# xultaeculcis/climate-super-resolution

Measured on NVIDIA B200. Metric: generator_inference_hr_mpixel_per_s, higher is better.
Workload: dtype bf16

## Files before the change

climate-super-resolution_b200/csrc/api.cu:

```cuda
#include <algorithm>
#include <atomic>
#include <cstdarg>
#include <cstdio>
#include <cstring>
#include <map>
#include <mutex>
#include <string>
#include <vector>

#include "../../include/climsr_b200.h"
#include "conv_tc.cuh"
#include "disc.cuh"
#include "elementwise.cuh"
#include "loss.cuh"
#include "metrics.cuh"
#include "rcan.cuh"
#include "rdb_tc.cuh"
#include "wgrad_tc.cuh"

namespace csr {

static thread_local char g_err[512] = "";
static std::atomic<long long> g_launches{0};
static int g_opt_pdl = 1;
// ... 9 lines not shown
static int g_opt_graphs = 1;
static int g_opt_graph_max_px = 1 << 21;
static int g_opt_wgrad_atomic = 1;
static int g_opt_eight_acc = 1;
static int g_opt_tall = 1;
static int g_opt_narrow_box = 1;
static int g_opt_trace_cta = 0;
static int g_opt_reserve_sms = 0;
static int g_opt_dense_min = 2;
static int g_opt_tap_pack = 1;
static int g_opt_hyb = 1;
static int g_opt_merge_phases = 1;
static int g_opt_fuse_tail = 3;
static int g_opt_dense = 1;
static int g_opt_early = 1;
static int g_dbg_wgrad[5] = {0, 0, 0, 0, 0};

static int fail(int code, const char* fmt, ...) {
  va_list ap;
  va_start(ap, fmt);
  vsnprintf(g_err, sizeof(g_err), fmt, ap);
  va_end(ap);
  return code;
}
#define CSR_CUDA(expr)                                                                          \
  do {                                                                                          \
    cudaError_t _e = (expr);                                                                    \
    if (_e != cudaSuccess) return fail(CSR_ERR_CUDA, "%s: %s", #expr, cudaGetErrorString(_e)); \
  } while (0)

// ... 160 lines not shown
        off = align_up(off + pp.npad * 4, 128);
        pl.parts.push_back(pp);
      }
    }
    out.push_back(pl);
  }
  *total = off;
  return out;
}

struct Tiling {
  int SW, TH, TW, win_rows, win_bytes, slot_bytes, n_slots, stage_bytes;
  double eff;
};
static int choose_tiling(int H, int W, int KH, int KW, int w_bytes, int n_kblocks, int stage_row_bytes, int n_stage, Tiling* out,
                         int row_bytes = 128, int tall = 1, int extra_slot_bytes = 0) {
  double best = -1;
  for (int SW = 16; SW <= 128; SW *= 2) {
    if (g_opt_force_sw && SW != g_opt_force_sw) continue;
    if (KW > 1 && SW > 32) continue;
    const int TW = SW - (KW - 1);
    if (TW < 1) continue;
    const int TH = kTileM / SW;
    const int win_rows = tall * TH + KH - 1;
    const int win_bytes = win_rows * SW * row_bytes;
    const int slot_bytes = (int)align_up(win_bytes, 1024) + (int)align_up(extra_slot_bytes, 1024);
    const int stage_bytes = stage_row_bytes ? (int)align_up((size_t)TH * TW * stage_row_bytes, 1024) : 0;
    const int fixed = 1024 + (int)align_up(w_bytes, 128) + 256 + 512 + n_stage * stage_bytes;
    const int slots = std::min(g_opt_max_slots, (kSmemLimit - fixed) / slot_bytes);
    if (slots < 1) continue;
    const double tiles = (double)ceil_div(H, TH * tall) * ceil_div(W, TW) * tall;
    double eff = (double)H * W / (tiles * kTileM);
    if (slots < std::min(2, n_kblocks + 1)) eff *= 0.7;
    eff -= 1e-4 * win_bytes / (double)(kTileM * 128);
    if (eff > best) {
      best = eff;
      *out = {SW, TH, TW, win_rows, win_bytes, slot_bytes, slots, stage_bytes, eff};
    }
  }
  if (best < 0) return fail(CSR_ERR_UNSUPPORTED, "no tile shape fits shared memory (weights %d bytes, %dx%d kernel)", w_bytes, KH, KW);
  return CSR_OK;
}

struct ConvLaunch {
  ConvParams p;
  CUtensorMap tmap;
  size_t w_off = 0, b_off = 0;
  size_t w2_off = 0, b2_off = 0;
};

struct DenseLaunch {
  DenseParams p;
  CUtensorMap tmap;
  size_t w_off[kDenseMaxLayers], b_off[kDenseMaxLayers];
// ... 70 lines not shown
    if (ok2 && te2.n_slots >= want) stages = 2;
    else if (ok1 && (!ok2 || te1.n_slots > te2.n_slots)) stages = 1;
    else if (ok2) stages = 2;
    const Tiling& te = stages == 1 ? te1 : te2;
    if (stages && te.n_slots >= std::min(2, p.n_kblocks + 1)) {
      tl = te;
      p.early = 1;
      p.n_groups = 1;
      p.n_stage = stages;
      if (4 * p.KW * p.npad <= 512 && !g_opt_two_acc) p.n_acc = 4;
    }
  }
  if (g_opt_hyb && p.early && ((p.KW == 3 && p.PW == 1) || (p.KW == 2 && p.PW <= 1)) && p.box_c == 64 && !p.stream_w) {
    p.hyb = 1;
    if (4 * (p.KW - 1) * p.npad <= 512 && !g_opt_two_acc) p.n_acc = 4;
  }
  p.SW = tl.SW; p.TH = tl.TH; p.TW = tl.TW;
  p.sw_shift = 0;
  while ((1 << p.sw_shift) < p.SW) ++p.sw_shift;
  p.tiles_x = ceil_div(W, p.TW);
  p.tiles_y = ceil_div(H, p.TH << p.tall_shift);
  p.num_tiles = p.tiles_x * p.tiles_y * N;
  p.tiles_per_img = p.tiles_x * p.tiles_y;
  if ((long long)p.tiles_x * p.tiles_y * N >= (1 << 24) || p.tiles_per_img >= (1 << 16))
    return fail(CSR_ERR_UNSUPPORTED, "too many tiles (%d x %d x %d) for one launch", p.tiles_x, p.tiles_y, N);
  p.magic_img = ((1ull << 40) / (unsigned)p.tiles_per_img) + 1;
  p.magic_row = ((1ull << 40) / (unsigned)p.tiles_x) + 1;
  p.win_rows = tl.win_rows; p.win_bytes = tl.win_bytes; p.slot_bytes = tl.slot_bytes; p.n_slots = tl.n_slots;
  p.win_slot_bytes = (int)align_up(tl.win_bytes, 1024);
  p.stage_bytes = tl.stage_bytes;
// ... 444 lines not shown
  int wmax = 0;
  for (int k = 0; k < 4; ++k) {
    const PackLayer& pl = packs[li + k];
    if (pl.parts.size() != 1 || pl.parts[0].npad != 16 || pl.parts[0].kh != 3 || pl.parts[0].kw != 3 || pl.cin_pad != nf + k * gc)
      return fail(CSR_ERR_UNSUPPORTED, "dense-block kernel: unexpected pack layout");
    p.L[k].ksteps = pl.cin_pad / 16;
    p.L[k].n_kblocks = ceil_div(pl.cin_pad, 64);
    p.L[k].w_bytes = pl.parts[0].w_bytes;
    p.L[k].out_coff = nf + k * gc;
    p.L[k].gate_coff = nf + (3 - k) * gc;
    dl->w_off[k] = pl.parts[0].w_off; dl->b_off[k] = pl.parts[0].b_off;
    wmax = std::max(wmax, pl.parts[0].w_bytes);
  }
  p.wbuf_bytes = (int)align_up(wmax, 1024);
  Tiling tl;
  int rc = choose_tiling(H, W, 3, 3, 2 * p.wbuf_bytes, 2, 32, 4, &tl, 128, 2);
  if (rc) return rc;
  if (tl.n_slots < 3) return fail(CSR_ERR_UNSUPPORTED, "dense-block kernel: window ring too shallow");
  p.SW = tl.SW; p.TH = tl.TH; p.TW = tl.TW;
  while ((1 << p.sw_shift) < p.SW) ++p.sw_shift;
  p.tiles_x = ceil_div(W, p.TW); p.tiles_y = ceil_div(H, 2 * p.TH);
  p.tiles_per_img = p.tiles_x * p.tiles_y;
  p.num_tiles = p.tiles_per_img * N;
  if ((long long)p.tiles_per_img * N >= (1 << 24) || p.tiles_per_img >= (1 << 16)) return fail(CSR_ERR_UNSUPPORTED, "dense-block kernel: too many windows");
  p.magic_img = ((1ull << 40) / (unsigned)p.tiles_per_img) + 1;
  p.magic_row = ((1ull << 40) / (unsigned)p.tiles_x) + 1;
  p.win_bytes = tl.win_bytes; p.slot_bytes = tl.slot_bytes; p.n_slots = std::min(tl.n_slots, 8);
  p.stage_bytes = (int)align_up((size_t)p.TH * p.TW * 32, 1024);
  if (dense_smem_bytes(p) > (size_t)kSmemLimit) return fail(CSR_ERR_UNSUPPORTED, "dense-block kernel needs %zu bytes of shared memory", dense_smem_bytes(p));
  return encode_act_map(&dl->tmap, buf, N, H, W, C, p.SW, 2 * p.TH + 2, 64);
}

static bool dense_enabled(const CsrNetDesc& d) { return g_opt_dense && d.gc == 16 && !g_opt_force_generic; }

static bool try_dense(const CsrPlan* P, const std::vector<PackLayer>& packs, int li, int j, void* buf, const void* gate, Op* op) {
  const CsrNetDesc& d = P->net;
  if (!dense_enabled(d)) return false;
  const size_t per_block = (size_t)kDenseMaxLayers * P->N * ceil_div(P->h, 8) * ceil_div(P->w, 14);
  op->kind = Op::kDense;
  return build_dense(packs, li, P->N, P->h, P->w, buf, P->ccat, d.nf, d.gc, P->flags + (size_t)j * per_block, &op->dense, gate, gate ? P->ccat : 0) ==
             CSR_OK &&
         (size_t)op->dense.p.num_tiles * kDenseMaxLayers <= per_block && op->dense.p.num_tiles >= g_opt_dense_min * P->sms;
}

static int plan_build(CsrPlan* P, const WsPtrs& ws, const std::vector<LayerSpec>& layers) {
  const CsrNetDesc& d = P->net;
  const int N = P->N, h = P->h, w = P->w;
  auto cat = [&](int j) -> void* { return ws.cat[P->train ? j : j % 3]; };
  size_t total = 0;
  const std::vector<PackLayer> packs = pack_layout(fwd_exec_table(d, layers), &total);
  const int C = P->ccat, nf = d.nf, gc = d.gc;
  std::vector<Op>& ops = P->fwd;
  {
    Op op; op.kind = Op::kNchw; op.dst = ws.xin; op.N = N; op.C = d.in_channels; op.H = h; op.W = w;
    ops.push_back(op);
  }
  int li = 0;
// ... 391 lines not shown
    case 2: g_opt_force_sw = value; return CSR_OK;
    case 3: g_opt_max_slots = value < 1 ? 1 : value; return CSR_OK;
    case 4: g_opt_no_tma_store = value ? 1 : 0; return CSR_OK;
    case 5: g_opt_two_acc = value ? 1 : 0; return CSR_OK;
    case 6: g_opt_force_generic = value ? 1 : 0; return CSR_OK;
    case 7: g_opt_one_mma = value ? 1 : 0; return CSR_OK;
    case 11: g_opt_graphs = value ? 1 : 0; return CSR_OK;
    case 12: g_opt_graph_max_px = value; return CSR_OK;
    case 15: g_opt_trace_cta = value; return CSR_OK;
    case 17: g_opt_narrow_box = value ? 1 : 0; return CSR_OK;
    case 18: g_opt_tall = value ? 1 : 0; return CSR_OK;
    case 19: g_opt_eight_acc = value ? 1 : 0; return CSR_OK;
    case 20: case 21: case 22: case 23: case 24: g_dbg_wgrad[key - 20] = value; return CSR_OK;
    case 25: g_opt_wgrad_atomic = value ? 1 : 0; return CSR_OK;
    case 27: g_opt_dense = value ? 1 : 0; return CSR_OK;
    case 36: g_opt_tap_pack = value ? 1 : 0; return CSR_OK;
    case 35:
      if (value != 0 && value != 1) return fail(CSR_ERR_BAD_ARG, "option 35: 0 or 1");
      g_opt_hyb = value; return CSR_OK;
    case 34: g_opt_merge_phases = value ? 1 : 0; return CSR_OK;
    case 33: g_opt_fuse_tail = value & 3; return CSR_OK;
    case 31: if (value < 0 || value > 64) return fail(CSR_ERR_BAD_ARG, "option 31: windows per SM in [0, 64]"); g_opt_dense_min = value; return CSR_OK;
    case 30: g_opt_reserve_sms = value < 0 ? 0 : value; return CSR_OK;
    case 26:
      if (value != 0 && value != 1) return fail(CSR_ERR_BAD_ARG, "option 26: 0 or 1");
      g_opt_early = value; return CSR_OK;
    default: return fail(CSR_ERR_BAD_ARG, "unknown option key %d", key);
  }
}

// ... 766 lines not shown
```

climate-super-resolution_b200/csrc/conv_tc.cu:

```cuda
#include <cstdio>

#include "conv_tc.cuh"
#include "ptx.cuh"

namespace csr {

namespace {

#ifdef CSR_ENABLE_TRACE
#define CSR_TRACE(role, tile_it, ev)                                                                                  \
  do {                                                                                                                \
    if (p.trace && blockIdx.x == p.trace_cta && (tile_it) < 64) p.trace[((role) * 64 + (tile_it)) * 8 + (ev)] = clock64();      \
  } while (0)
#else
#define CSR_TRACE(role, tile_it, ev) do { } while (0)
#endif

struct Tile {
  int n, y0, x0;
};

__device__ __forceinline__ int fast_div(int t, unsigned long long magic) {
  return static_cast<int>((static_cast<unsigned long long>(static_cast<unsigned>(t)) * magic) >> 40);
}
// ... 32 lines not shown
#pragma unroll
    for (int j = 0; j < 8; ++j) s[j] = __uint_as_float(raw[j]);
  } else {
    const int src = (lane + delta) & 31;
#pragma unroll
    for (int j = 0; j < 8; ++j) s[j] = __uint_as_float(__shfl_sync(0xffffffffu, raw[j], src));
  }
#pragma unroll
  for (int j = 0; j < 8; j += 2) {
    const float2 t = __fadd2_rn(make_float2(acc[j], acc[j + 1]), make_float2(s[j], s[j + 1]));
    acc[j] = t.x;
    acc[j + 1] = t.y;
  }
}

__device__ __forceinline__ void fma_residual8(float (&v)[8], const uint4& r, float scale) {
  const uint32_t w[4] = {r.x, r.y, r.z, r.w};
#pragma unroll
  for (int i = 0; i < 4; ++i) {
    const float2 t = __ffma2_rn(make_float2(v[2 * i], v[2 * i + 1]), make_float2(scale, scale), make_float2(bf16lo(w[i]), bf16hi(w[i])));
    v[2 * i] = t.x;
    v[2 * i + 1] = t.y;
  }
}

__device__ __forceinline__ void gate8(float (&v)[8], const uint4& g, float neg) {
  const uint32_t w[4] = {g.x, g.y, g.z, g.w};
#pragma unroll
  for (int i = 0; i < 4; ++i) {
    v[2 * i] *= (bf16lo(w[i]) > 0.f) ? 1.f : neg;
    v[2 * i + 1] *= (bf16hi(w[i]) > 0.f) ? 1.f : neg;
  }
}

__device__ __forceinline__ uint4 ldg16(const void* base, size_t pix, int C, int coff) {
  return __ldg(reinterpret_cast<const uint4*>(reinterpret_cast<const __nv_bfloat16*>(base) + pix * C + coff));
}

}

template <int KW_T, int PW_T, int ACT_T, int RES_T, int ST_T, int TALL_T = 0, int EARLY_T = 0, int FUSE_T = 0, int HYB_T = 0>
__global__ void __launch_bounds__(kConvThreads, 1)
conv_tc_kernel(const ConvParams p, const __grid_constant__ CUtensorMap tmap) {
  static_assert(!HYB_T || EARLY_T, "hybrid tap fold: early-release epilogue only");
  extern __shared__ uint8_t smem_raw[];
  const uint32_t smem_base = (smem_u32(smem_raw) + 1023u) & ~1023u;
  const uint32_t slots_addr = smem_base;
  const uint32_t stage_addr = slots_addr + static_cast<uint32_t>(p.n_slots) * p.slot_bytes;
  const uint32_t w_addr = stage_addr + static_cast<uint32_t>(p.n_stage) * p.stage_bytes;
  const int w_local = p.stream_w ? 0 : p.w_bytes;
  const uint32_t w2_addr = w_addr + ((w_local + 127) & ~127);
  const uint32_t b2_addr = w2_addr + (FUSE_T ? static_cast<uint32_t>(p.w2_bytes) : 0u);
  const uint32_t bias_addr = b2_addr + (FUSE_T ? 128u : 0u);
  const uint32_t bar_addr = bias_addr + 256;
  const int S = p.n_slots;
  const int NA = p.n_acc;
  const int NG = p.n_groups;
  const int wpg = kEpilogueWarps / NG;
  auto bar_w = bar_addr;
// ... 72 lines not shown
        if (kb == 0 && lane == 0) CSR_TRACE(0, pit, 0);
        mbar_wait_spin(bar_a_empty(slot), phase ^ 1);
        if (kb == 0 && lane == 0) CSR_TRACE(0, pit, 1);
        if (elect_one()) {
          if (p.stream_w) {
            const int ks_here = min(4, (p.cin >> 4) - kb * 4);
            const int wbytes = p.KH * ks_here * (KW * p.npad) * 32;
            mbar_arrive_expect_tx(bar_a_full(slot), p.win_bytes + wbytes);
            const uint8_t* wsrc = reinterpret_cast<const uint8_t*>(p.wpk) + static_cast<size_t>(blockIdx.y) * p.part_w_bytes +
                                  static_cast<size_t>(kb) * p.wkb_bytes;
            const uint32_t wdst = slots_addr + slot * p.slot_bytes + p.win_slot_bytes;
            for (int off = 0; off < wbytes; off += 32768) bulk_load(wdst + off, wsrc + off, min(32768, wbytes - off), bar_a_full(slot));
          } else {
            mbar_arrive_expect_tx(bar_a_full(slot), p.win_bytes);
          }
          tma_load_4d(slots_addr + slot * p.slot_bytes, &tmap, bar_a_full(slot), p.cin_off + kb * 64, tl.x0 - p.PW, tl.y0 - ph_eff, tl.n);
        }
        __syncwarp();
        if (++slot == S) { slot = 0; phase ^= 1; }
      }
    }
  } else if (warp <= kMmaWarps) {
    if (warp > p.n_mma) goto done;
    const int mw = warp - 1;
    const uint32_t idesc = make_idesc_bf16(kTileM, nmma);
    const uint32_t b_step16 = static_cast<uint32_t>(nmma * 32) >> 4;
    const uint32_t kb_w16 = static_cast<uint32_t>(p.KH * 4) * b_step16;
    const uint32_t row_bytes = static_cast<uint32_t>(p.box_c) * 2u;
    const uint32_t row16 = static_cast<uint32_t>(p.SW) * (row_bytes >> 4);
    const uint32_t a_layout = p.box_c == 64 ? 2u : p.box_c == 32 ? 4u : 6u;
    const uint32_t a_hi = ((8u * row_bytes) >> 4) | (1u << 14) | (a_layout << 29);
// ... 90 lines not shown
    }
  } else {
    const int ew = warp - 1 - kMmaWarps;
    const int g = ew / wpg;
    const int wj = ew - g * wpg;
    const int lane_grp = warp & 3;
    const int sub = wj >> 2;
    const int cstep = wpg >> 2;
    const int gthreads = wpg * 32;
    const bool tracer = (ew == 0 && lane == 0);
    const int m = lane_grp * 32 + lane;
    const int ty = m >> p.sw_shift;
    const int tx = m & (p.SW - 1);
    const int n_chunks = ST_T == 3 ? 1 : p.npad >> 3;
    const int PW = KW_T ? PW_T : p.PW;
    const bool col_ok = (tx >= PW) && (tx < PW + p.TW);
    const int srow = ty * p.TW + (tx - PW);
    const int act = ACT_T >= 0 ? ACT_T : p.act;
    const bool has_r1 = RES_T >= 0 ? (RES_T & 1) != 0 : p.r1 != nullptr;
    const bool has_r2 = RES_T >= 0 ? (RES_T & 2) != 0 : p.r2 != nullptr;
    const bool has_gate = RES_T >= 0 ? (RES_T & 4) != 0 : p.gate != nullptr;
    const bool tma_store = ST_T >= 0 ? ST_T == 1 : (p.store_mode == kStoreStaged);
    const bool need_pix = !tma_store || has_r1 || has_r2 || has_gate;
    const uint32_t swz = (p.stage_row_bytes == 128) ? static_cast<uint32_t>(srow & 7) : 0u;
    const uint32_t srow_addr = stage_addr + static_cast<uint32_t>(g) * p.stage_bytes + static_cast<uint32_t>(srow * p.stage_row_bytes);
    const uint32_t sbuf = stage_addr + static_cast<uint32_t>(g) * p.stage_bytes;
    const uint32_t t_lane = tmem_base + (static_cast<uint32_t>(lane_grp * 32) << 16);
    const int d0 = -PW, d1 = 1 - PW, d2 = 2 - PW;
    const int rp = p.stage_row_bytes >> 4;
    const int n_pieces = p.TH * p.TW * rp;
    uint32_t pc_s[4], pc_d[4], pc_yx[4];
    if (tma_store) {
      const int tid_g = wj * 32 + lane;
#pragma unroll
      for (int k = 0; k < 4; ++k) {
        const int i = tid_g + k * gthreads;
        const int sr = i / rp, c = i - sr * rp;
        const int dy = sr / p.TW, dx = sr - dy * p.TW;
        const uint32_t z = (p.stage_row_bytes == 128) ? static_cast<uint32_t>(sr & 7) : 0u;
        pc_s[k] = sbuf + static_cast<uint32_t>(sr * p.stage_row_bytes) + ((static_cast<uint32_t>(c) ^ z) << 4);
        pc_d[k] = static_cast<uint32_t>((dy * p.out_sy * p.out_W + dx * p.out_sx) * p.out_C + c * 8);
// ... 149 lines not shown
        }
      }
    } else
    for (int it = g; ; it += NG) {
      const int t = blockIdx.x + (it >> TALL_T) * static_cast<int>(gridDim.x);
      if (t >= p.num_tiles) break;
      if (tracer) CSR_TRACE(2, it, 3);
      Tile tl = decode_tile<TALL_T>(p, t);
      if constexpr (TALL_T) tl.y0 += (it & 1) * p.TH;
      bool valid = false;
      size_t pix = 0;
      int y = 0, x = 0;
      uint4 q1[4], q2[4];
      if (need_pix) {
        y = tl.y0 + ty;
        x = tl.x0 - PW + tx;
        valid = col_ok && (y < p.H) && (x < p.W);
        pix = (static_cast<size_t>(tl.n) * p.H + y) * p.W + x;
#pragma unroll
        for (int j = 0; j < 4; ++j) {
          const int ch0 = (2 * (sub + (j >> 1) * cstep) + (j & 1)) * 8;
          const bool on = valid && (ch0 < p.n_store);
          q1[j] = (on && has_r1) ? ldg16(p.r1, pix, p.r1_C, p.r1_coff + ch0) : make_uint4(0, 0, 0, 0);
          if (has_gate)
            q2[j] = (on && ch0 >= p.gate_from) ? ldg16(p.gate, pix, p.gate_C, p.gate_coff + ch0)
                                               : make_uint4(0x3f803f80u, 0x3f803f80u, 0x3f803f80u, 0x3f803f80u);
          else
            q2[j] = (on && has_r2) ? ldg16(p.r2, pix, p.r2_C, p.r2_coff + ch0) : make_uint4(0, 0, 0, 0);
        }
      }
      if (tma_store) named_bar_sync(1 + g, gthreads);
// ... 19 lines not shown
            tmem_ld_wait();
            gather_add8(v, r0, 0, lane);
          } else if constexpr (KW_T == 2) {
            uint32_t r0[8], r1[8];
            tmem_ld8(t_addr + ch0, r0);
            tmem_ld8(t_addr + p.npad + ch0, r1);
            tmem_ld_wait();
            gather_add8(v, r0, d0, lane);
            gather_add8(v, r1, d1, lane);
          } else if constexpr (KW_T == 3) {
            uint32_t r0[8], r1[8], r2[8];
            tmem_ld8(t_addr + ch0, r0);
            tmem_ld8(t_addr + p.npad + ch0, r1);
            tmem_ld8(t_addr + 2 * p.npad + ch0, r2);
            tmem_ld_wait();
            gather_add8(v, r0, d0, lane);
            gather_add8(v, r1, d1, lane);
            gather_add8(v, r2, d2, lane);
          } else {
            for (int dx = 0; dx < KW; ++dx) {
              uint32_t r[8];
              tmem_ld8(t_addr + dx * p.npad + ch0, r);
              tmem_ld_wait();
              gather_add8(v, r, dx - PW, lane);
            }
          }
          apply_act8(v, act, p.act_slope);
          if (need_pix) {
            if (has_r1) fma_residual8(v, q1[j], p.s1);
            if (has_gate) gate8(v, q2[j], p.gate_neg);
            else if (has_r2) fma_residual8(v, q2[j], p.s2);
          }
          if (tma_store) {
// ... 50 lines not shown
  __syncthreads();
  timeline_end(p.timeline, p.launch_id);
  if (warp == 1) {
    __syncwarp();
    tc_fence_after();
    tmem_dealloc(tmem_base, p.tmem_cols);
  }
}

size_t conv_smem_bytes(const ConvParams& p) {
  return 1024  + static_cast<size_t>(p.n_slots) * p.slot_bytes + static_cast<size_t>(p.n_stage) * p.stage_bytes +
         (((p.stream_w ? 0 : p.w_bytes) + 127) & ~127) + (p.fuse2 ? p.w2_bytes + 128 : 0) + 256  +
         8 * (18 + 2 * p.n_slots) + 32;
}

template <int KW_T, int PW_T, int ACT_T, int RES_T, int ST_T, int TALL_T = 0, int EARLY_T = 0, int FUSE_T = 0, int HYB_T = 0>
static int launch_t(const ConvParams& p, const CUtensorMap& tmap, int num_sms, cudaStream_t stream) {
  const size_t smem = conv_smem_bytes(p);
  if (smem > static_cast<size_t>(kSmemLimit)) return static_cast<int>(cudaErrorInvalidValue);
  static bool configured[64] = {};
  auto kern = conv_tc_kernel<KW_T, PW_T, ACT_T, RES_T, ST_T, TALL_T, EARLY_T, FUSE_T, HYB_T>;
  int dev = 0;
  if (cudaGetDevice(&dev) != cudaSuccess || dev < 0 || dev >= 64) return static_cast<int>(cudaErrorInvalidDevice);
  if (!configured[dev]) {
    cudaError_t e = cudaFuncSetAttribute(kern, cudaFuncAttributeMaxDynamicSharedMemorySize, kSmemLimit);
    if (e != cudaSuccess) return static_cast<int>(e);
    configured[dev] = true;
  }
  cudaLaunchConfig_t cfg{};
  const int parts = p.parts > 1 ? p.parts : 1;
  const int per_part = num_sms / parts > 0 ? num_sms / parts : 1;
  cfg.gridDim = dim3(p.num_tiles < per_part ? p.num_tiles : per_part, parts);
  cfg.blockDim = dim3(kConvThreads);
  cfg.dynamicSmemBytes = smem;
  cfg.stream = stream;
  cudaLaunchAttribute attr[1];
  attr[0].id = cudaLaunchAttributeProgrammaticStreamSerialization;
  attr[0].val.programmaticStreamSerializationAllowed = p.use_pdl ? 1 : 0;
  cfg.attrs = attr;
  cfg.numAttrs = 1;
  return static_cast<int>(cudaLaunchKernelEx(&cfg, kern, p, tmap));
}

int launch_conv_tc(const ConvParams& p, const CUtensorMap& tmap, int num_sms, cudaStream_t stream) {
  const int res = (p.r1 ? 1 : 0) | (p.r2 ? 2 : 0) | (p.gate ? 4 : 0);
  if ((res & 6) == 6) return static_cast<int>(cudaErrorInvalidValue);
  if (p.tall_shift) {
    if ((p.n_acc != 4 && p.n_acc != 8) || p.n_groups != 4) return static_cast<int>(cudaErrorInvalidValue);
    if (p.store_mode == kStoreStaged && !p.force_generic && p.KW == 3 && p.PW == 1 && p.act == 1 && res == 0)
      return launch_t<3, 1, 1, 0, 1, 1>(p, tmap, num_sms, stream);
    if (p.store_mode == kStoreStaged && !p.force_generic && p.KW == 1 && p.PW == 0 && p.act == 2 && res == 0)
      return launch_t<1, 0, 2, 0, 1, 1>(p, tmap, num_sms, stream);
    if (p.store_mode == kStoreStaged && !p.force_generic && p.KW == 3 && p.PW == 1 && p.act == 0 && res == 4)
      return launch_t<3, 1, 0, 4, 1, 1>(p, tmap, num_sms, stream);
    if (p.store_mode == kStoreStaged && !p.force_generic && p.KW == 3 && p.PW == 1 && p.act == 0 && res == 5)
      return launch_t<3, 1, 0, 5, 1, 1>(p, tmap, num_sms, stream);
    if (p.store_mode == kStoreStaged && !p.force_generic && p.KW == 1 && p.PW == 0 && p.act == 0 && res == 4)
      return launch_t<1, 0, 0, 4, 1, 1>(p, tmap, num_sms, stream);
    if (p.store_mode == kStoreF32Planar && !p.force_generic && p.KW == 3 && p.PW == 1 && p.act == 0 && res == 0)
      return launch_t<3, 1, 0, 0, 3, 1>(p, tmap, num_sms, stream);
    if (p.store_mode == kStoreF32Planar && !p.force_generic && p.KW == 5 && p.PW == 2 && p.act == 0 && res == 0)
// ... 67 lines not shown
```

climate-super-resolution_b200/csrc/conv_tc.cuh:

```cuda
#pragma once
#include <cuda.h>
#include <cuda_runtime.h>
#include <stdint.h>

namespace csr {

constexpr int kEpilogueWarps = 16;
constexpr int kEpilogueThreads = kEpilogueWarps * 32;
constexpr int kMmaWarps = 2;
constexpr int kConvThreads = 32 * (1 + kMmaWarps) + kEpilogueThreads;
constexpr int kTileM = 128;
constexpr int kSmemLimit = 232448;
constexpr int kMaxNpad = 64;

enum StoreMode {
  kStoreStaged = 0,
  kStoreDirect = 1,
  kStoreF32Planar = 2,
  kStoreF32Nhwc = 3
};

struct ConvParams {
  int N, H, W;
  int KH, KW, PH, PW;
// ... 13 lines not shown
  int n_mma;
  int n_acc;
  int n_groups;
  int n_stage;
  int hyb;
  int early;
  int tmem_cols;
  int force_generic;
  int trace_cta;
  int box_c;
  int tall_shift;
  int stream_w;
  int wkb_bytes;
  int win_slot_bytes;
  int use_pdl;
  int parts, part_w_bytes, part_b_floats, part_c;
  int part_ph, part_oy;
  int fuse2, w2_bytes, n2;
  const void* w2;
  const float* b2;
  void* out2; int out2_C, out2_coff;
  long long out2_plane;
  const float* bias;
  const void* wpk;
  int act;
  float act_slope;
  float s1, s2;
  const void* r1; int r1_C, r1_coff;
  const void* r2; int r2_C, r2_coff;
  const void* gate; int gate_C, gate_coff; int gate_from; float gate_neg;
// ... 17 lines not shown
```

climate-super-resolution_b200/csrc/rdb_tc.cu:

```cuda
#include <cstdio>

#include "conv_tc.cuh"
#include "ptx.cuh"
#include "rdb_tc.cuh"

namespace csr {

namespace {

constexpr int kNpad = 16;
constexpr int kNmma = 3 * kNpad;
constexpr int kAcc = 8;
constexpr int kGroups = 4;

struct Win {
  int n, y0, x0, ty, tx;
};

__device__ __forceinline__ int fast_div(int t, unsigned long long magic) {
  return static_cast<int>((static_cast<unsigned long long>(static_cast<unsigned>(t)) * magic) >> 40);
}
__device__ __forceinline__ Win decode_win(const DenseParams& p, int t) {
  Win r;
  r.n = fast_div(t, p.magic_img);
// ... 26 lines not shown
#pragma unroll
    for (int j = 0; j < 8; ++j) s[j] = __uint_as_float(raw[j]);
  } else {
    const int src = (lane + delta) & 31;
#pragma unroll
    for (int j = 0; j < 8; ++j) s[j] = __uint_as_float(__shfl_sync(0xffffffffu, raw[j], src));
  }
#pragma unroll
  for (int j = 0; j < 8; j += 2) {
    const float2 t = __fadd2_rn(make_float2(acc[j], acc[j + 1]), make_float2(s[j], s[j + 1]));
    acc[j] = t.x;
    acc[j + 1] = t.y;
  }
}

}

__global__ void __launch_bounds__(kConvThreads, 1)
dense_block_kernel(const DenseParams p, const __grid_constant__ CUtensorMap tmap) {
  extern __shared__ uint8_t smem_raw[];
  const uint32_t smem_base = (smem_u32(smem_raw) + 1023u) & ~1023u;
  const int S = p.n_slots;
  const uint32_t slots_addr = smem_base;
  const uint32_t stage_addr = slots_addr + static_cast<uint32_t>(S) * p.slot_bytes;
  const uint32_t w_addr = stage_addr + static_cast<uint32_t>(kGroups) * p.stage_bytes;
  const uint32_t bias_addr = w_addr + 2u * p.wbuf_bytes;
  const uint32_t bar_addr = bias_addr + kDenseMaxLayers * kNpad * 4;
  auto bar_w_full = [&](int b) { return bar_addr + 8u * b; };
  auto bar_w_free = [&](int b) { return bar_addr + 8u * (2 + b); };
  auto bar_a_full = [&](int s) { return bar_addr + 8u * (4 + s); };
  auto bar_a_empty = [&](int s) { return bar_addr + 8u * (4 + S + s); };
  auto bar_acc_full = [&](int b) { return bar_addr + 8u * (4 + 2 * S + b); };
  auto bar_acc_empty = [&](int b) { return bar_addr + 8u * (4 + 2 * S + kAcc + b); };
  const uint32_t tmem_slot_addr = bar_addr + 8u * (4 + 2 * S + 2 * kAcc);
  uint8_t* smem_gen = smem_raw + (smem_base - smem_u32(smem_raw));
  float* bias_s = reinterpret_cast<float*>(smem_gen + (bias_addr - smem_base));
  volatile uint32_t* tmem_slot = reinterpret_cast<volatile uint32_t*>(smem_gen + (tmem_slot_addr - smem_base));
  volatile uint32_t* progress = tmem_slot + 1;

  const int warp = threadIdx.x >> 5;
  const int lane = threadIdx.x & 31;
  const int nl = p.n_layers;

  griddep_launch_dependents();

  if (threadIdx.x == 0) {
    progress[0] = 0;
    progress[1] = 0;
    tma_prefetch_desc(&tmap);
// ... 11 lines not shown
    }
    fence_mbar_init();
    fence_proxy_async_smem();
    for (int l = 0; l < 2 && l < nl; ++l) {
      mbar_arrive_expect_tx(bar_w_full(l), p.L[l].w_bytes);
      const uint8_t* wsrc = reinterpret_cast<const uint8_t*>(p.L[l].wpk);
      for (int off = 0; off < p.L[l].w_bytes; off += 32768)
        bulk_load(w_addr + l * p.wbuf_bytes + off, wsrc + off, min(32768, p.L[l].w_bytes - off), bar_w_full(l));
    }
  }
  if (warp == 1) {
    tmem_alloc(tmem_slot_addr, 512);
    tmem_relinquish();
  }
  for (int i = threadIdx.x; i < nl * kNpad; i += blockDim.x) bias_s[i] = p.L[i / kNpad].bias[i % kNpad];
  tc_fence_before();
  __syncthreads();
  tc_fence_after();
  const uint32_t tmem_base = *tmem_slot;

  griddep_wait();
  timeline_start(p.timeline, p.launch_id);

  const int G = static_cast<int>(gridDim.x);
  const int nwin = (p.num_tiles - static_cast<int>(blockIdx.x) + G - 1) / G;

  if (warp == 0) {
    int slot = 0;
    uint32_t phase = 0;
    for (int l = 0; l < nl; ++l) {
// ... 8 lines not shown
              const int idx = w.n * p.tiles_per_img + yy * p.tiles_x + xx;
              unsigned have, spins = 0;
              while ((have = ld_acquire_gpu(fl + idx)) < 2u) {
                if (++spins > (1u << 24)) flag_timeout(l - 1, idx, have);
                __nanosleep(40);
              }
            }
          }
          __syncwarp();
          fence_proxy_async_all();
        }
        for (int kb = 0; kb < p.L[l].n_kblocks; ++kb) {
          mbar_wait_spin(bar_a_empty(slot), phase ^ 1);
          if (elect_one()) {
            mbar_arrive_expect_tx(bar_a_full(slot), p.win_bytes);
            tma_load_4d(slots_addr + slot * p.slot_bytes, &tmap, bar_a_full(slot), kb * 64, w.x0 - 1, w.y0 - 1, w.n);
          }
          __syncwarp();
          if (++slot == S) { slot = 0; phase ^= 1; }
        }
      }
      if (l >= 1 && l + 1 < nl) {
        const int b = (l + 1) & 1;
        mbar_wait_spin(bar_w_free(b), static_cast<uint32_t>((l - 1) >> 1) & 1u);
        if (elect_one()) {
          mbar_arrive_expect_tx(bar_w_full(b), p.L[l + 1].w_bytes);
          const uint8_t* wsrc = reinterpret_cast<const uint8_t*>(p.L[l + 1].wpk);
          for (int off = 0; off < p.L[l + 1].w_bytes; off += 32768)
            bulk_load(w_addr + b * p.wbuf_bytes + off, wsrc + off, min(32768, p.L[l + 1].w_bytes - off), bar_w_full(b));
        }
        __syncwarp();
// ... 67 lines not shown
          __syncwarp();
          if (++slot == S) { slot = 0; phase ^= 1; }
        }
      }
      if (elect_one()) umma_commit(bar_w_free(l & 1));
      __syncwarp();
    }
  } else {
    const int ew = warp - 1 - kMmaWarps;
    const int g = ew >> 2;
    const int wj = ew & 3;
    const int lane_grp = warp & 3;
    const int m_row = lane_grp * 32 + lane;
    const int ty = m_row >> p.sw_shift;
    const int tx = m_row & (p.SW - 1);
    const bool col_ok = (tx >= 1) && (tx < 1 + p.TW);
    const int srow = ty * p.TW + (tx - 1);
    const uint32_t sbuf = stage_addr + static_cast<uint32_t>(g) * p.stage_bytes;
    const uint32_t srow_addr = sbuf + static_cast<uint32_t>(srow * 32);
    const uint32_t t_lane = tmem_base + (static_cast<uint32_t>(lane_grp * 32) << 16);
    const int n_pieces = p.TH * p.TW * 2;
    uint32_t pc_s[2], pc_d[2], pc_yx[2];
#pragma unroll
    for (int k = 0; k < 2; ++k) {
      const int i = wj * 32 + lane + k * 128;
      const int sr = i >> 1, c = i & 1;
      const int dy = sr / p.TW, dx = sr - dy * p.TW;
      pc_s[k] = sbuf + static_cast<uint32_t>(sr * 32 + c * 16);
      pc_d[k] = static_cast<uint32_t>((dy * p.W + dx) * p.C + c * 8);
      pc_yx[k] = (i < n_pieces) ? ((static_cast<uint32_t>(dy) << 16) | static_cast<uint32_t>(dx)) : 0xffffffffu;
    }
    const int m_total = 2 * nwin * nl;
    int l = 0, it = g >> 1;
    while (it >= nwin && l < nl) { it -= nwin; ++l; }
    for (int m = g; m < m_total; m += kGroups) {
      const int half = m & 1;
      const int buf = m & 7;
      const uint32_t acc_par = (static_cast<uint32_t>(m) >> 3) & 1u;
      const int t = blockIdx.x + it * G;
      const Win w = decode_win(p, t);
      const int y0 = w.y0 + half * p.TH;
      const uint32_t t_addr = t_lane + buf * kNmma;
      uint4 gq[2] = {make_uint4(0x3f803f80u, 0x3f803f80u, 0x3f803f80u, 0x3f803f80u), make_uint4(0x3f803f80u, 0x3f803f80u, 0x3f803f80u, 0x3f803f80u)};
      if (p.gate) {
        const int y = y0 + ty, x = w.x0 - 1 + tx;
        if (col_ok && y < p.H && x < p.W) {
          const uint4* gsrc = reinterpret_cast<const uint4*>(reinterpret_cast<const __nv_bfloat16*>(p.gate) +
                                                             ((static_cast<size_t>(w.n) * p.H + y) * p.W + x) * p.gate_C + p.L[l].gate_coff);
          gq[0] = __ldg(gsrc);
          gq[1] = __ldg(gsrc + 1);
        }
      }
      mbar_wait(bar_acc_full(buf), acc_par);
      tc_fence_after();
      uint32_t raw[2][3][8];
#pragma unroll
      for (int jj = 0; jj < 2; ++jj)
#pragma unroll
        for (int dx = 0; dx < 3; ++dx) tmem_ld8(t_addr + dx * kNpad + jj * 8, raw[jj][dx]);
      tmem_ld_wait();
      tc_fence_before();
      __syncwarp();
      if (lane == 0) mbar_arrive(bar_acc_empty(buf));
#pragma unroll
      for (int jj = 0; jj < 2; ++jj) {
        float v[8];
        {
          const float4 b0 = *reinterpret_cast<const float4*>(bias_s + l * kNpad + jj * 8);
          const float4 b1 = *reinterpret_cast<const float4*>(bias_s + l * kNpad + jj * 8 + 4);
          v[0] = b0.x; v[1] = b0.y; v[2] = b0.z; v[3] = b0.w; v[4] = b1.x; v[5] = b1.y; v[6] = b1.z; v[7] = b1.w;
        }
        gather_add8(v, raw[jj][0], -1, lane);
        gather_add8(v, raw[jj][1], 0, lane);
        gather_add8(v, raw[jj][2], 1, lane);
        if (p.act) {
#pragma unroll
          for (int j = 0; j < 8; j += 2) {
            const float2 s2 = __fmul2_rn(make_float2(v[j], v[j + 1]), make_float2(0.2f, 0.2f));
            v[j] = fmaxf(v[j], s2.x);
            v[j + 1] = fmaxf(v[j + 1], s2.y);
          }
        }
        if (p.gate) {
          const uint32_t gw[4] = {gq[jj].x, gq[jj].y, gq[jj].z, gq[jj].w};
#pragma unroll
          for (int i = 0; i < 4; ++i) {
            v[2 * i] *= (bf16lo(gw[i]) > 0.f) ? 1.f : p.gate_neg;
            v[2 * i + 1] *= (bf16hi(gw[i]) > 0.f) ? 1.f : p.gate_neg;
          }
// ... 23 lines not shown
    }
  }

  tc_fence_before();
  __syncthreads();
  timeline_end(p.timeline, p.launch_id);
  if (warp == 1) {
    __syncwarp();
    tc_fence_after();
    tmem_dealloc(tmem_base, 512);
  }
}

size_t dense_smem_bytes(const DenseParams& p) {
  return 1024 + static_cast<size_t>(p.n_slots) * p.slot_bytes + static_cast<size_t>(kGroups) * p.stage_bytes + 2u * p.wbuf_bytes +
         kDenseMaxLayers * kNpad * 4 + 8 * (4 + 2 * p.n_slots + 2 * kAcc) + 32;
}

int launch_dense_block(const DenseParams& p, const CUtensorMap& tmap, int num_sms, cudaStream_t stream) {
  const size_t smem = dense_smem_bytes(p);
  if (smem > static_cast<size_t>(kSmemLimit) || p.n_layers < 1 || p.n_layers > kDenseMaxLayers || p.n_slots < 2)
    return static_cast<int>(cudaErrorInvalidValue);
  static bool configured[64] = {};
  int dev = 0;
  if (cudaGetDevice(&dev) != cudaSuccess || dev < 0 || dev >= 64) return static_cast<int>(cudaErrorInvalidDevice);
  if (!configured[dev]) {
    cudaError_t e = cudaFuncSetAttribute(dense_block_kernel, cudaFuncAttributeMaxDynamicSharedMemorySize, kSmemLimit);
    if (e != cudaSuccess) return static_cast<int>(e);
    configured[dev] = true;
  }
  cudaLaunchConfig_t cfg{};
  cfg.gridDim = dim3(p.num_tiles < num_sms ? p.num_tiles : num_sms);
  cfg.blockDim = dim3(kConvThreads);
  cfg.dynamicSmemBytes = smem;
  cfg.stream = stream;
  cudaLaunchAttribute attr[1];
  attr[0].id = cudaLaunchAttributeProgrammaticStreamSerialization;
  attr[0].val.programmaticStreamSerializationAllowed = p.use_pdl ? 1 : 0;
  cfg.attrs = attr;
  cfg.numAttrs = 1;
  return static_cast<int>(cudaLaunchKernelEx(&cfg, dense_block_kernel, p, tmap));
}

}
```

climate-super-resolution_b200/csrc/rdb_tc.cuh:

```cuda
#pragma once
#include <cuda.h>
#include <cuda_runtime.h>
#include <stdint.h>

namespace csr {

constexpr int kDenseMaxLayers = 4;

struct DenseLayerParams {
  int ksteps;
  int n_kblocks;
  int w_bytes;
  int out_coff;
  const void* wpk;
  const float* bias;
  int gate_coff;
};

struct DenseParams {
  int N, H, W;
  int SW, sw_shift, TH, TW;
  int tiles_x, tiles_y, num_tiles, tiles_per_img;
  unsigned long long magic_img, magic_row;
  int win_bytes;
  int slot_bytes;
  int n_slots;
  int stage_bytes;
  int wbuf_bytes;
  int n_layers;
  int C;
  void* buf;
  unsigned int* flags;
  int use_pdl;
  int act;
  const void* gate;
  int gate_C;
// ... 11 lines not shown
```

Measured before the change: 948.0.

## Use full-row tiles without column halo for narrow-width 3x3 convs and dense blocks

When the image width is 16, 32 or 64, conv and dense-block tiles now span the whole row, so the window is loaded without the left/right halo columns. Edge pixels take zero padding from a masked shuffle, and for 64-wide dense tiles the values at the 32-lane warp boundary are passed through shared memory behind a named barrier. This removes the wasted halo columns, which otherwise cost 2 of every 16 or 32 tile positions. It adds a template variant, an exchange buffer and extra synchronisation in the epilogue. Dense-block flag sizing is now computed from the actual tile count.

```diff
diff --git a/climate-super-resolution_b200/csrc/api.cu b/climate-super-resolution_b200/csrc/api.cu
--- a/climate-super-resolution_b200/csrc/api.cu
+++ b/climate-super-resolution_b200/csrc/api.cu
@@ -47,6 +47,7 @@
 static int g_opt_fuse_tail = 3;
 static int g_opt_dense = 1;
 static int g_opt_early = 1;
+static int g_opt_full_row = 1;
 static int g_dbg_wgrad[5] = {0, 0, 0, 0, 0};
 
 static int fail(int code, const char* fmt, ...) {
@@ -237,12 +238,13 @@
   double eff;
 };
 static int choose_tiling(int H, int W, int KH, int KW, int w_bytes, int n_kblocks, int stage_row_bytes, int n_stage, Tiling* out,
-                         int row_bytes = 128, int tall = 1, int extra_slot_bytes = 0) {
+                         int row_bytes = 128, int tall = 1, int extra_slot_bytes = 0, bool full_row = false) {
   double best = -1;
   for (int SW = 16; SW <= 128; SW *= 2) {
     if (g_opt_force_sw && SW != g_opt_force_sw) continue;
-    if (KW > 1 && SW > 32) continue;
-    const int TW = SW - (KW - 1);
+    if (full_row && SW != W) continue;
+    if (KW > 1 && SW > (full_row ? 64 : 32)) continue;
+    const int TW = full_row ? SW : SW - (KW - 1);
     if (TW < 1) continue;
     const int TH = kTileM / SW;
     const int win_rows = tall * TH + KH - 1;
@@ -261,6 +263,7 @@
       *out = {SW, TH, TW, win_rows, win_bytes, slot_bytes, slots, stage_bytes, eff};
     }
   }
+  if (best < 0 && full_row) return CSR_ERR_UNSUPPORTED;
   if (best < 0) return fail(CSR_ERR_UNSUPPORTED, "no tile shape fits shared memory (weights %d bytes, %dx%d kernel)", w_bytes, KH, KW);
   return CSR_OK;
 }
@@ -361,6 +364,17 @@
   if (g_opt_hyb && p.early && ((p.KW == 3 && p.PW == 1) || (p.KW == 2 && p.PW <= 1)) && p.box_c == 64 && !p.stream_w) {
     p.hyb = 1;
     if (4 * (p.KW - 1) * p.npad <= 512 && !g_opt_two_acc) p.n_acc = 4;
+  }
+  const int res = (io.r1 ? 1 : 0) | (io.r2 ? 2 : 0) | (io.gate ? 4 : 0);
+  if (g_opt_full_row && (W == 16 || W == 32) && pp.kh == 3 && p.KW == 3 && p.PW == 1 && pp.ph == 1 && up == 1 && p.act == CSR_ACT_NONE &&
+      (res == 1 || res == 3 || res == 4 || res == 5) && tma_out && !p.tall_shift && !p.early && !p.stream_w && p.box_c == 64 &&
+      !g_opt_force_generic) {
+    Tiling tf;
+    if (choose_tiling(H, W, 3, 3, p.w_bytes, p.n_kblocks, p.stage_row_bytes, p.n_groups, &tf, 128, 1, 0, true) == CSR_OK &&
+        tf.n_slots >= std::min(2, p.n_kblocks + 1)) {
+      tl = tf;
+      p.full_row = 1;
+    }
   }
   p.SW = tl.SW; p.TH = tl.TH; p.TW = tl.TW;
   p.sw_shift = 0;
@@ -835,8 +849,14 @@
   }
   p.wbuf_bytes = (int)align_up(wmax, 1024);
   Tiling tl;
-  int rc = choose_tiling(H, W, 3, 3, 2 * p.wbuf_bytes, 2, 32, 4, &tl, 128, 2);
-  if (rc) return rc;
+  if (g_opt_full_row && (W == 16 || W == 32 || W == 64) &&
+      choose_tiling(H, W, 3, 3, 2 * p.wbuf_bytes + 1072, 2, 32, 4, &tl, 128, 2, 0, true) == CSR_OK &&
+      tl.n_slots >= 3)
+    p.full_row = 1;
+  else {
+    int rc = choose_tiling(H, W, 3, 3, 2 * p.wbuf_bytes, 2, 32, 4, &tl, 128, 2);
+    if (rc) return rc;
+  }
   if (tl.n_slots < 3) return fail(CSR_ERR_UNSUPPORTED, "dense-block kernel: window ring too shallow");
   p.SW = tl.SW; p.TH = tl.TH; p.TW = tl.TW;
   while ((1 << p.sw_shift) < p.SW) ++p.sw_shift;
@@ -857,11 +877,12 @@
 static bool try_dense(const CsrPlan* P, const std::vector<PackLayer>& packs, int li, int j, void* buf, const void* gate, Op* op) {
   const CsrNetDesc& d = P->net;
   if (!dense_enabled(d)) return false;
-  const size_t per_block = (size_t)kDenseMaxLayers * P->N * ceil_div(P->h, 8) * ceil_div(P->w, 14);
   op->kind = Op::kDense;
-  return build_dense(packs, li, P->N, P->h, P->w, buf, P->ccat, d.nf, d.gc, P->flags + (size_t)j * per_block, &op->dense, gate, gate ? P->ccat : 0) ==
-             CSR_OK &&
-         (size_t)op->dense.p.num_tiles * kDenseMaxLayers <= per_block && op->dense.p.num_tiles >= g_opt_dense_min * P->sms;
+  if (build_dense(packs, li, P->N, P->h, P->w, buf, P->ccat, d.nf, d.gc, nullptr, &op->dense, gate, gate ? P->ccat : 0) != CSR_OK) return false;
+  const size_t per_block = (size_t)kDenseMaxLayers * op->dense.p.num_tiles;
+  if ((j + 1) * per_block * sizeof(unsigned int) > P->flags_bytes) return false;
+  op->dense.p.flags = P->flags + (size_t)j * per_block;
+  return op->dense.p.num_tiles >= g_opt_dense_min * P->sms;
 }
 
 static int plan_build(CsrPlan* P, const WsPtrs& ws, const std::vector<LayerSpec>& layers) {
@@ -1283,6 +1304,7 @@
     case 20: case 21: case 22: case 23: case 24: g_dbg_wgrad[key - 20] = value; return CSR_OK;
     case 25: g_opt_wgrad_atomic = value ? 1 : 0; return CSR_OK;
     case 27: g_opt_dense = value ? 1 : 0; return CSR_OK;
+    case 37: g_opt_full_row = value ? 1 : 0; return CSR_OK;
     case 36: g_opt_tap_pack = value ? 1 : 0; return CSR_OK;
     case 35:
       if (value != 0 && value != 1) return fail(CSR_ERR_BAD_ARG, "option 35: 0 or 1");
diff --git a/climate-super-resolution_b200/csrc/conv_tc.cu b/climate-super-resolution_b200/csrc/conv_tc.cu
--- a/climate-super-resolution_b200/csrc/conv_tc.cu
+++ b/climate-super-resolution_b200/csrc/conv_tc.cu
@@ -70,6 +70,22 @@
   }
 }
 
+__device__ __forceinline__ void gather_add8_edge(float (&acc)[8], const uint32_t (&raw)[8], int delta, int lane, bool edge) {
+  float s[8];
+  const int src = (lane + delta) & 31;
+#pragma unroll
+  for (int j = 0; j < 8; ++j) {
+    const float nb = __uint_as_float(__shfl_sync(0xffffffffu, raw[j], src));
+    s[j] = edge ? 0.f : nb;
+  }
+#pragma unroll
+  for (int j = 0; j < 8; j += 2) {
+    const float2 t = __fadd2_rn(make_float2(acc[j], acc[j + 1]), make_float2(s[j], s[j + 1]));
+    acc[j] = t.x;
+    acc[j + 1] = t.y;
+  }
+}
+
 __device__ __forceinline__ void fma_residual8(float (&v)[8], const uint4& r, float scale) {
   const uint32_t w[4] = {r.x, r.y, r.z, r.w};
 #pragma unroll
@@ -95,10 +111,11 @@
 
 }
 
-template <int KW_T, int PW_T, int ACT_T, int RES_T, int ST_T, int TALL_T = 0, int EARLY_T = 0, int FUSE_T = 0, int HYB_T = 0>
+template <int KW_T, int PW_T, int ACT_T, int RES_T, int ST_T, int TALL_T = 0, int EARLY_T = 0, int FUSE_T = 0, int HYB_T = 0, int FR_T = 0>
 __global__ void __launch_bounds__(kConvThreads, 1)
 conv_tc_kernel(const ConvParams p, const __grid_constant__ CUtensorMap tmap) {
   static_assert(!HYB_T || EARLY_T, "hybrid tap fold: early-release epilogue only");
+  static_assert(!FR_T || (KW_T == 3 && PW_T == 1 && ST_T == 1 && !TALL_T && !EARLY_T), "full-row tiles: 3x3 staged single-tile layers");
   extern __shared__ uint8_t smem_raw[];
   const uint32_t smem_base = (smem_u32(smem_raw) + 1023u) & ~1023u;
   const uint32_t slots_addr = smem_base;
@@ -201,7 +218,8 @@
           } else {
             mbar_arrive_expect_tx(bar_a_full(slot), p.win_bytes);
           }
-          tma_load_4d(slots_addr + slot * p.slot_bytes, &tmap, bar_a_full(slot), p.cin_off + kb * 64, tl.x0 - p.PW, tl.y0 - ph_eff, tl.n);
+          tma_load_4d(slots_addr + slot * p.slot_bytes, &tmap, bar_a_full(slot), p.cin_off + kb * 64, tl.x0 - (FR_T ? 0 : p.PW), tl.y0 - ph_eff,
+                      tl.n);
         }
         __syncwarp();
         if (++slot == S) { slot = 0; phase ^= 1; }
@@ -322,8 +340,9 @@
     const int tx = m & (p.SW - 1);
     const int n_chunks = ST_T == 3 ? 1 : p.npad >> 3;
     const int PW = KW_T ? PW_T : p.PW;
-    const bool col_ok = (tx >= PW) && (tx < PW + p.TW);
-    const int srow = ty * p.TW + (tx - PW);
+    const int xoff = FR_T ? 0 : PW;
+    const bool col_ok = FR_T || ((tx >= PW) && (tx < PW + p.TW));
+    const int srow = ty * p.TW + (tx - xoff);
     const int act = ACT_T >= 0 ? ACT_T : p.act;
     const bool has_r1 = RES_T >= 0 ? (RES_T & 1) != 0 : p.r1 != nullptr;
     const bool has_r2 = RES_T >= 0 ? (RES_T & 2) != 0 : p.r2 != nullptr;
@@ -333,6 +352,7 @@
     const uint32_t swz = (p.stage_row_bytes == 128) ? static_cast<uint32_t>(srow & 7) : 0u;
     const uint32_t srow_addr = stage_addr + static_cast<uint32_t>(g) * p.stage_bytes + static_cast<uint32_t>(srow * p.stage_row_bytes);
     const uint32_t sbuf = stage_addr + static_cast<uint32_t>(g) * p.stage_bytes;
+    const bool edge0 = FR_T && tx == 0, edge2 = FR_T && tx == p.SW - 1;
     const uint32_t t_lane = tmem_base + (static_cast<uint32_t>(lane_grp * 32) << 16);
     const int d0 = -PW, d1 = 1 - PW, d2 = 2 - PW;
     const int rp = p.stage_row_bytes >> 4;
@@ -512,7 +532,7 @@
       uint4 q1[4], q2[4];
       if (need_pix) {
         y = tl.y0 + ty;
-        x = tl.x0 - PW + tx;
+        x = tl.x0 - xoff + tx;
         valid = col_ok && (y < p.H) && (x < p.W);
         pix = (static_cast<size_t>(tl.n) * p.H + y) * p.W + x;
 #pragma unroll
@@ -562,9 +582,15 @@
             tmem_ld8(t_addr + p.npad + ch0, r1);
             tmem_ld8(t_addr + 2 * p.npad + ch0, r2);
             tmem_ld_wait();
-            gather_add8(v, r0, d0, lane);
-            gather_add8(v, r1, d1, lane);
-            gather_add8(v, r2, d2, lane);
+            if constexpr (FR_T) {
+              gather_add8_edge(v, r0, -1, lane, edge0);
+              gather_add8(v, r1, 0, lane);
+              gather_add8_edge(v, r2, 1, lane, edge2);
+            } else {
+              gather_add8(v, r0, d0, lane);
+              gather_add8(v, r1, d1, lane);
+              gather_add8(v, r2, d2, lane);
+            }
           } else {
             for (int dx = 0; dx < KW; ++dx) {
               uint32_t r[8];
@@ -645,12 +671,12 @@
          8 * (18 + 2 * p.n_slots) + 32;
 }
 
-template <int KW_T, int PW_T, int ACT_T, int RES_T, int ST_T, int TALL_T = 0, int EARLY_T = 0, int FUSE_T = 0, int HYB_T = 0>
+template <int KW_T, int PW_T, int ACT_T, int RES_T, int ST_T, int TALL_T = 0, int EARLY_T = 0, int FUSE_T = 0, int HYB_T = 0, int FR_T = 0>
 static int launch_t(const ConvParams& p, const CUtensorMap& tmap, int num_sms, cudaStream_t stream) {
   const size_t smem = conv_smem_bytes(p);
   if (smem > static_cast<size_t>(kSmemLimit)) return static_cast<int>(cudaErrorInvalidValue);
   static bool configured[64] = {};
-  auto kern = conv_tc_kernel<KW_T, PW_T, ACT_T, RES_T, ST_T, TALL_T, EARLY_T, FUSE_T, HYB_T>;
+  auto kern = conv_tc_kernel<KW_T, PW_T, ACT_T, RES_T, ST_T, TALL_T, EARLY_T, FUSE_T, HYB_T, FR_T>;
   int dev = 0;
   if (cudaGetDevice(&dev) != cudaSuccess || dev < 0 || dev >= 64) return static_cast<int>(cudaErrorInvalidDevice);
   if (!configured[dev]) {
@@ -676,6 +702,18 @@
 int launch_conv_tc(const ConvParams& p, const CUtensorMap& tmap, int num_sms, cudaStream_t stream) {
   const int res = (p.r1 ? 1 : 0) | (p.r2 ? 2 : 0) | (p.gate ? 4 : 0);
   if ((res & 6) == 6) return static_cast<int>(cudaErrorInvalidValue);
+  if (p.full_row) {
+    if (p.store_mode != kStoreStaged || p.force_generic || p.KW != 3 || p.PW != 1 || p.act != 0 || p.tall_shift || p.early || p.stream_w ||
+        (p.SW != 16 && p.SW != 32) || p.SW != p.W || p.TW != p.SW || p.tiles_x != 1 || p.n_stage != p.n_groups)
+      return static_cast<int>(cudaErrorInvalidValue);
+    switch (res) {
+      case 1: return launch_t<3, 1, 0, 1, 1, 0, 0, 0, 0, 1>(p, tmap, num_sms, stream);
+      case 3: return launch_t<3, 1, 0, 3, 1, 0, 0, 0, 0, 1>(p, tmap, num_sms, stream);
+      case 4: return launch_t<3, 1, 0, 4, 1, 0, 0, 0, 0, 1>(p, tmap, num_sms, stream);
+      case 5: return launch_t<3, 1, 0, 5, 1, 0, 0, 0, 0, 1>(p, tmap, num_sms, stream);
+      default: return static_cast<int>(cudaErrorInvalidValue);
+    }
+  }
   if (p.tall_shift) {
     if ((p.n_acc != 4 && p.n_acc != 8) || p.n_groups != 4) return static_cast<int>(cudaErrorInvalidValue);
     if (p.store_mode == kStoreStaged && !p.force_generic && p.KW == 3 && p.PW == 1 && p.act == 1 && res == 0)
diff --git a/climate-super-resolution_b200/csrc/conv_tc.cuh b/climate-super-resolution_b200/csrc/conv_tc.cuh
--- a/climate-super-resolution_b200/csrc/conv_tc.cuh
+++ b/climate-super-resolution_b200/csrc/conv_tc.cuh
@@ -51,6 +51,7 @@
   int wkb_bytes;
   int win_slot_bytes;
   int use_pdl;
+  int full_row;
   int parts, part_w_bytes, part_b_floats, part_c;
   int part_ph, part_oy;
   int fuse2, w2_bytes, n2;
diff --git a/climate-super-resolution_b200/csrc/rdb_tc.cu b/climate-super-resolution_b200/csrc/rdb_tc.cu
--- a/climate-super-resolution_b200/csrc/rdb_tc.cu
+++ b/climate-super-resolution_b200/csrc/rdb_tc.cu
@@ -64,8 +64,26 @@
   }
 }
 
-}
-
+__device__ __forceinline__ void gather_add8_edge(float (&acc)[8], const uint32_t (&raw)[8], int delta, int lane, bool edge, uint32_t ext) {
+  uint32_t s[8];
+  const int src = (lane + delta) & 31;
+#pragma unroll
+  for (int j = 0; j < 8; ++j) s[j] = __shfl_sync(0xffffffffu, raw[j], src);
+  if (edge) {
+    const uint4 e0 = ld_shared_v4(ext), e1 = ld_shared_v4(ext + 16);
+    s[0] = e0.x; s[1] = e0.y; s[2] = e0.z; s[3] = e0.w; s[4] = e1.x; s[5] = e1.y; s[6] = e1.z; s[7] = e1.w;
+  }
+#pragma unroll
+  for (int j = 0; j < 8; j += 2) {
+    const float2 t = __fadd2_rn(make_float2(acc[j], acc[j + 1]), make_float2(__uint_as_float(s[j]), __uint_as_float(s[j + 1])));
+    acc[j] = t.x;
+    acc[j + 1] = t.y;
+  }
+}
+
+}
+
+template <int FR_T>
 __global__ void __launch_bounds__(kConvThreads, 1)
 dense_block_kernel(const DenseParams p, const __grid_constant__ CUtensorMap tmap) {
   extern __shared__ uint8_t smem_raw[];
@@ -83,6 +101,7 @@
   auto bar_acc_full = [&](int b) { return bar_addr + 8u * (4 + 2 * S + b); };
   auto bar_acc_empty = [&](int b) { return bar_addr + 8u * (4 + 2 * S + kAcc + b); };
   const uint32_t tmem_slot_addr = bar_addr + 8u * (4 + 2 * S + 2 * kAcc);
+  const uint32_t xch_addr = (tmem_slot_addr + 31u) & ~15u;
   uint8_t* smem_gen = smem_raw + (smem_base - smem_u32(smem_raw));
   float* bias_s = reinterpret_cast<float*>(smem_gen + (bias_addr - smem_base));
   volatile uint32_t* tmem_slot = reinterpret_cast<volatile uint32_t*>(smem_gen + (tmem_slot_addr - smem_base));
@@ -124,6 +143,7 @@
     tmem_relinquish();
   }
   for (int i = threadIdx.x; i < nl * kNpad; i += blockDim.x) bias_s[i] = p.L[i / kNpad].bias[i % kNpad];
+  if (FR_T && threadIdx.x < 8) reinterpret_cast<uint32_t*>(smem_gen + (xch_addr - smem_base))[threadIdx.x] = 0u;
   tc_fence_before();
   __syncthreads();
   tc_fence_after();
@@ -162,7 +182,7 @@
           mbar_wait_spin(bar_a_empty(slot), phase ^ 1);
           if (elect_one()) {
             mbar_arrive_expect_tx(bar_a_full(slot), p.win_bytes);
-            tma_load_4d(slots_addr + slot * p.slot_bytes, &tmap, bar_a_full(slot), kb * 64, w.x0 - 1, w.y0 - 1, w.n);
+            tma_load_4d(slots_addr + slot * p.slot_bytes, &tmap, bar_a_full(slot), kb * 64, w.x0 - (FR_T ? 0 : 1), w.y0 - 1, w.n);
           }
           __syncwarp();
           if (++slot == S) { slot = 0; phase ^= 1; }
@@ -260,8 +280,13 @@
     const int m_row = lane_grp * 32 + lane;
     const int ty = m_row >> p.sw_shift;
     const int tx = m_row & (p.SW - 1);
-    const bool col_ok = (tx >= 1) && (tx < 1 + p.TW);
-    const int srow = ty * p.TW + (tx - 1);
+    constexpr int xoff = FR_T ? 0 : 1;
+    const bool col_ok = FR_T || ((tx >= 1) && (tx < 1 + p.TW));
+    const int srow = ty * p.TW + (tx - xoff);
+    const bool sw64 = FR_T && p.SW == 64;
+    const uint32_t xch_pair = xch_addr + 32u + static_cast<uint32_t>(g * 2 + (lane_grp >> 1)) * 128u;
+    const bool xthread = sw64 && (tx == 31 || tx == 32);
+    const bool edge0 = FR_T && (tx == 0 || tx == 32), edge2 = FR_T && (tx == p.SW - 1 || tx == 31);
     const uint32_t sbuf = stage_addr + static_cast<uint32_t>(g) * p.stage_bytes;
     const uint32_t srow_addr = sbuf + static_cast<uint32_t>(srow * 32);
     const uint32_t t_lane = tmem_base + (static_cast<uint32_t>(lane_grp * 32) << 16);
@@ -289,7 +314,7 @@
       const uint32_t t_addr = t_lane + buf * kNmma;
       uint4 gq[2] = {make_uint4(0x3f803f80u, 0x3f803f80u, 0x3f803f80u, 0x3f803f80u), make_uint4(0x3f803f80u, 0x3f803f80u, 0x3f803f80u, 0x3f803f80u)};
       if (p.gate) {
-        const int y = y0 + ty, x = w.x0 - 1 + tx;
+        const int y = y0 + ty, x = w.x0 - xoff + tx;
         if (col_ok && y < p.H && x < p.W) {
           const uint4* gsrc = reinterpret_cast<const uint4*>(reinterpret_cast<const __nv_bfloat16*>(p.gate) +
                                                              ((static_cast<size_t>(w.n) * p.H + y) * p.W + x) * p.gate_C + p.L[l].gate_coff);
@@ -308,6 +333,21 @@
       tc_fence_before();
       __syncwarp();
       if (lane == 0) mbar_arrive(bar_acc_empty(buf));
+      if (sw64) {
+        if (tx == 31) {
+          st_shared_v4(xch_pair, raw[0][0][0], raw[0][0][1], raw[0][0][2], raw[0][0][3]);
+          st_shared_v4(xch_pair + 16, raw[0][0][4], raw[0][0][5], raw[0][0][6], raw[0][0][7]);
+          st_shared_v4(xch_pair + 32, raw[1][0][0], raw[1][0][1], raw[1][0][2], raw[1][0][3]);
+          st_shared_v4(xch_pair + 48, raw[1][0][4], raw[1][0][5], raw[1][0][6], raw[1][0][7]);
+        }
+        if (tx == 32) {
+          st_shared_v4(xch_pair + 64, raw[0][2][0], raw[0][2][1], raw[0][2][2], raw[0][2][3]);
+          st_shared_v4(xch_pair + 80, raw[0][2][4], raw[0][2][5], raw[0][2][6], raw[0][2][7]);
+          st_shared_v4(xch_pair + 96, raw[1][2][0], raw[1][2][1], raw[1][2][2], raw[1][2][3]);
+          st_shared_v4(xch_pair + 112, raw[1][2][4], raw[1][2][5], raw[1][2][6], raw[1][2][7]);
+        }
+        named_bar_sync(5 + g * 2 + (lane_grp >> 1), 64);
+      }
 #pragma unroll
       for (int jj = 0; jj < 2; ++jj) {
         float v[8];
@@ -316,9 +356,16 @@
           const float4 b1 = *reinterpret_cast<const float4*>(bias_s + l * kNpad + jj * 8 + 4);
           v[0] = b0.x; v[1] = b0.y; v[2] = b0.z; v[3] = b0.w; v[4] = b1.x; v[5] = b1.y; v[6] = b1.z; v[7] = b1.w;
         }
-        gather_add8(v, raw[jj][0], -1, lane);
-        gather_add8(v, raw[jj][1], 0, lane);
-        gather_add8(v, raw[jj][2], 1, lane);
+        if constexpr (FR_T) {
+          const uint32_t ext = xthread ? xch_pair + (tx == 31 ? 64u : 0u) + jj * 32u : xch_addr;
+          gather_add8_edge(v, raw[jj][0], -1, lane, edge0, ext);
+          gather_add8(v, raw[jj][1], 0, lane);
+          gather_add8_edge(v, raw[jj][2], 1, lane, edge2, ext);
+        } else {
+          gather_add8(v, raw[jj][0], -1, lane);
+          gather_add8(v, raw[jj][1], 0, lane);
+          gather_add8(v, raw[jj][2], 1, lane);
+        }
         if (p.act) {
 #pragma unroll
           for (int j = 0; j < 8; j += 2) {
@@ -372,20 +419,23 @@
 
 size_t dense_smem_bytes(const DenseParams& p) {
   return 1024 + static_cast<size_t>(p.n_slots) * p.slot_bytes + static_cast<size_t>(kGroups) * p.stage_bytes + 2u * p.wbuf_bytes +
-         kDenseMaxLayers * kNpad * 4 + 8 * (4 + 2 * p.n_slots + 2 * kAcc) + 32;
+         kDenseMaxLayers * kNpad * 4 + 8 * (4 + 2 * p.n_slots + 2 * kAcc) + 32 + (p.full_row ? 16 + 32 + 1024 : 0);
 }
 
 int launch_dense_block(const DenseParams& p, const CUtensorMap& tmap, int num_sms, cudaStream_t stream) {
   const size_t smem = dense_smem_bytes(p);
   if (smem > static_cast<size_t>(kSmemLimit) || p.n_layers < 1 || p.n_layers > kDenseMaxLayers || p.n_slots < 2)
     return static_cast<int>(cudaErrorInvalidValue);
-  static bool configured[64] = {};
+  if (p.full_row && ((p.SW != 16 && p.SW != 32 && p.SW != 64) || p.SW != p.W || p.TW != p.SW || p.tiles_x != 1))
+    return static_cast<int>(cudaErrorInvalidValue);
+  auto kern = p.full_row ? dense_block_kernel<1> : dense_block_kernel<0>;
+  static bool configured[2][64] = {};
   int dev = 0;
   if (cudaGetDevice(&dev) != cudaSuccess || dev < 0 || dev >= 64) return static_cast<int>(cudaErrorInvalidDevice);
-  if (!configured[dev]) {
-    cudaError_t e = cudaFuncSetAttribute(dense_block_kernel, cudaFuncAttributeMaxDynamicSharedMemorySize, kSmemLimit);
+  if (!configured[p.full_row][dev]) {
+    cudaError_t e = cudaFuncSetAttribute(kern, cudaFuncAttributeMaxDynamicSharedMemorySize, kSmemLimit);
     if (e != cudaSuccess) return static_cast<int>(e);
-    configured[dev] = true;
+    configured[p.full_row][dev] = true;
   }
   cudaLaunchConfig_t cfg{};
   cfg.gridDim = dim3(p.num_tiles < num_sms ? p.num_tiles : num_sms);
@@ -397,7 +447,7 @@
   attr[0].val.programmaticStreamSerializationAllowed = p.use_pdl ? 1 : 0;
   cfg.attrs = attr;
   cfg.numAttrs = 1;
-  return static_cast<int>(cudaLaunchKernelEx(&cfg, dense_block_kernel, p, tmap));
-}
-
-}
+  return static_cast<int>(cudaLaunchKernelEx(&cfg, kern, p, tmap));
+}
+
+}
diff --git a/climate-super-resolution_b200/csrc/rdb_tc.cuh b/climate-super-resolution_b200/csrc/rdb_tc.cuh
--- a/climate-super-resolution_b200/csrc/rdb_tc.cuh
+++ b/climate-super-resolution_b200/csrc/rdb_tc.cuh
@@ -20,6 +20,7 @@
 struct DenseParams {
   int N, H, W;
   int SW, sw_shift, TH, TW;
+  int full_row;
   int tiles_x, tiles_y, num_tiles, tiles_per_img;
   unsigned long long magic_img, magic_row;
   int win_bytes;
```

Result: faster. 1000 (median of 6 runs) (+5.5%).
